# multi-template-matching/MultiTemplateMatching-Python

Measured on AMD Instinct MI355X. Metric: Mpixel-correlations/s, higher is better.
Workload: dtype u8

## Files before the change

include/mtm_hip.h:

```cpp
#ifndef MTM_HIP_H
#define MTM_HIP_H

#include <stddef.h>
#include <stdint.h>

#ifdef __cplusplus
extern "C" {
#endif

#define MTM_ABI_VERSION 9

#define MTM_U8  0
#define MTM_F32 1
#define MTM_U16 2

#define MTM_TM_SQDIFF        0
#define MTM_TM_SQDIFF_NORMED 1
#define MTM_TM_CCORR         2
#define MTM_TM_CCORR_NORMED  3
#define MTM_TM_CCOEFF        4
#define MTM_TM_CCOEFF_NORMED 5

#define MTM_PEAKS_LOCAL  0
#define MTM_PEAKS_GLOBAL 1
// ... 61 lines not shown
    int32_t kernel_used;
    int64_t n_hits;
    int32_t hits_only;
    float   sclk_mhz;
    float   ncc_sum_ms;
    int32_t f32_route;
    int32_t sq_launches;
    float   masked_stat_ms;
    int32_t f32_pieces;
} mtm_timing;

int         mtm_abi_version(void);
int         mtm_device_count(void);
const char* mtm_last_error(void);
int         mtm_ctx_create(mtm_ctx** out, int device_id);
void        mtm_ctx_destroy(mtm_ctx* ctx);
int         mtm_set_option(mtm_ctx* ctx, int option, int64_t value);
int         mtm_get_option(mtm_ctx* ctx, int option, int64_t* value);
#define MTM_POISON_SCRATCH 1
#define MTM_POISON_LDS     2
#define MTM_POISON_ARENAS  4
int         mtm_debug_poison(mtm_ctx* ctx, int pattern_byte, int what);
int         mtm_debug_quotient_check(mtm_ctx* ctx, uint64_t n_cases, uint64_t seed, uint64_t* out4);
void*       mtm_host_alloc(size_t bytes);
void        mtm_host_free(void* p);

int mtm_set_image(mtm_ctx* ctx, const void* px, int rows, int cols, int chans, int dtype,
                  int64_t row_stride_bytes);
int mtm_set_image_downscaled(mtm_ctx* ctx, const void* px, int rows, int cols, int chans, int dtype,
                             int64_t row_stride_bytes, int factor);

int mtm_set_templates(mtm_ctx* ctx, const mtm_templ* templs, int n_templ, int method);

typedef struct mtm_variant {
    int32_t rot90;
    int32_t flip_lr;
    int32_t flip_ud;
    int32_t rows, cols;
    int32_t down;
} mtm_variant;
int mtm_set_templates_augmented(mtm_ctx* ctx, const mtm_templ* bases, int n_bases,
                                const mtm_variant* variants, int n_variants, int method);

int mtm_score_map(mtm_ctx* ctx, int templ_idx, float* out, int64_t out_row_stride_bytes);

int mtm_find_matches(mtm_ctx* ctx, int mode, double score_threshold,
// ... 98 lines not shown
```

multitemplatematching-python_amd/MTM/_lib.py:

```python
import ctypes
import struct
import os
import threading
import weakref

import numpy as np

_HERE = os.path.dirname(os.path.abspath(__file__))
LIB_PATH = os.environ.get("MTM_LIB_PATH") or os.path.join(_HERE, "libmtm_hip.so")

MTM_U8, MTM_F32, MTM_U16 = 0, 1, 2
GROUP_EXCHANGE_HOST, GROUP_EXCHANGE_RCCL = 0, 1
PEAKS_LOCAL, PEAKS_GLOBAL = 0, 1
BORDER_CONSTANT, BORDER_NEAREST = 0, 1
KERNEL_AUTO, KERNEL_NAIVE, KERNEL_DOT4, KERNEL_MFMA = 0, 1, 2, 3
OPT_KERNEL, OPT_PEAK_BORDER, OPT_HIT_CAPACITY, OPT_DOT4_VARIANT, OPT_EXACT_DIV, OPT_HITS_ONLY, OPT_F32_MFMA = 1, 2, 3, 4, 5, 6, 7
OPT_BATCH_MAX_ROWS = 8
OPT_BOXES_MAX_FLOATS = 9
ALL_OPTIONS = (OPT_KERNEL, OPT_PEAK_BORDER, OPT_HIT_CAPACITY, OPT_DOT4_VARIANT, OPT_EXACT_DIV, OPT_HITS_ONLY, OPT_F32_MFMA,
               OPT_BATCH_MAX_ROWS, OPT_BOXES_MAX_FLOATS)
BATCH_MAX_ROWS = 65535
POISON_SCRATCH, POISON_LDS, POISON_ARENAS = 1, 2, 4
E_OVERFLOW = -5
E_HIP = -2
# ... 25 lines not shown

HIT_DTYPE = np.dtype([("templ_idx", "<i4"), ("x", "<i4"), ("y", "<i4"), ("w", "<i4"), ("h", "<i4"),
                      ("score", "<f4")])
BOX_UNIT_DTYPE = np.dtype([("templ_idx", "<i4"), ("y0", "<i4"), ("x0", "<i4"), ("rows", "<i4"), ("cols", "<i4")])
POINT_DTYPE = np.dtype([("templ_idx", "<i4"), ("x", "<i4"), ("y", "<i4")])
assert HIT_DTYPE.itemsize == ctypes.sizeof(MtmHit) == 24
TEMPL_DTYPE = np.dtype([("px", "<u8"), ("mask", "<u8"), ("rows", "<i4"), ("cols", "<i4"), ("chans", "<i4"),
                        ("dtype", "<i4"), ("row_stride", "<i8"), ("mask_row_stride", "<i8")])
assert TEMPL_DTYPE.itemsize == ctypes.sizeof(MtmTempl) == 48
VARIANT_DTYPE = np.dtype([("rot90", "<i4"), ("flip_lr", "<i4"), ("flip_ud", "<i4"), ("rows", "<i4"), ("cols", "<i4"),
                          ("down", "<i4")])

_P = ctypes.POINTER
SYMBOLS = {
    "mtm_abi_version": (ctypes.c_int, []),
    "mtm_device_count": (ctypes.c_int, []),
    "mtm_last_error": (ctypes.c_char_p, []),
    "mtm_ctx_create": (ctypes.c_int, [_P(ctypes.c_void_p), ctypes.c_int]),
    "mtm_ctx_destroy": (None, [ctypes.c_void_p]),
    "mtm_set_option": (ctypes.c_int, [ctypes.c_void_p, ctypes.c_int, ctypes.c_int64]),
    "mtm_get_option": (ctypes.c_int, [ctypes.c_void_p, ctypes.c_int, _P(ctypes.c_int64)]),
    "mtm_debug_poison": (ctypes.c_int, [ctypes.c_void_p, ctypes.c_int, ctypes.c_int]),
    "mtm_debug_quotient_check": (ctypes.c_int, [ctypes.c_void_p, ctypes.c_uint64, ctypes.c_uint64, _P(ctypes.c_uint64)]),
    "mtm_set_image": (ctypes.c_int, [ctypes.c_void_p, ctypes.c_void_p, ctypes.c_int, ctypes.c_int,
                                     ctypes.c_int, ctypes.c_int, ctypes.c_int64]),
    "mtm_set_image_downscaled": (ctypes.c_int, [ctypes.c_void_p, ctypes.c_void_p, ctypes.c_int, ctypes.c_int, ctypes.c_int,
                                                ctypes.c_int, ctypes.c_int64, ctypes.c_int]),
    "mtm_set_templates": (ctypes.c_int, [ctypes.c_void_p, ctypes.c_void_p, ctypes.c_int, ctypes.c_int]),
    "mtm_set_templates_augmented": (ctypes.c_int, [ctypes.c_void_p, ctypes.c_void_p, ctypes.c_int, ctypes.c_void_p, ctypes.c_int,
                                                   ctypes.c_int]),
    "mtm_score_map": (ctypes.c_int, [ctypes.c_void_p, ctypes.c_int, ctypes.c_void_p, ctypes.c_int64]),
    "mtm_find_matches": (ctypes.c_int, [ctypes.c_void_p, ctypes.c_int, ctypes.c_double, ctypes.c_void_p,
                                        ctypes.c_int64, _P(ctypes.c_int64)]),
    "mtm_find_matches_image": (ctypes.c_int, [ctypes.c_void_p, ctypes.c_void_p, ctypes.c_int, ctypes.c_int, ctypes.c_int,
                                              ctypes.c_int, ctypes.c_int64, ctypes.c_int, ctypes.c_double, ctypes.c_void_p,
                                              ctypes.c_int64, _P(ctypes.c_int64)]),
    "mtm_find_matches_image_nms": (ctypes.c_int, [ctypes.c_void_p, ctypes.c_void_p, ctypes.c_int, ctypes.c_int, ctypes.c_int,
                                                  ctypes.c_int, ctypes.c_int64, ctypes.c_double, ctypes.c_double, ctypes.c_int64,
                                                  ctypes.c_void_p, ctypes.c_int64, _P(ctypes.c_int64)]),
    "mtm_find_matches_image_sharded_nms": (ctypes.c_int, [ctypes.c_void_p, ctypes.c_void_p, ctypes.c_int, ctypes.c_int, ctypes.c_int,
                                                          ctypes.c_int, ctypes.c_int64, ctypes.c_double, ctypes.c_double,
                                                          ctypes.c_int64, ctypes.c_int, ctypes.c_void_p, ctypes.c_int,
                                                          ctypes.c_void_p, ctypes.c_int64, _P(ctypes.c_int64)]),
    "mtm_find_matches_batch": (ctypes.c_int, [ctypes.c_void_p, ctypes.c_void_p, ctypes.c_int, ctypes.c_int, ctypes.c_int,
                                              ctypes.c_int, ctypes.c_int, ctypes.c_int64, ctypes.c_int, ctypes.c_double,
                                              ctypes.c_void_p, ctypes.c_int64, ctypes.c_void_p, _P(ctypes.c_int64)]),
# ... 209 lines not shown

class _RecordMemo:
    _rec_key = _rec = _rec_keep = _rec_src = None

    def _records(self, templates):
        if type(templates) is FrozenUnits and templates is self._rec_src and self._rec_key is not None:
            return self._rec
        key = [(id(t), t.shape, id(m)) for t, m in templates]
        if key != self._rec_key:
            self._rec, keep = templ_records(templates)
            self._rec_keep = (keep, [t for t, _ in templates], [m for _, m in templates])
            self._rec_key = key if _zero_copy(templates, keep) else None
        self._rec_src = templates
        return self._rec


_LIVE = weakref.WeakSet()


def live_contexts():
    return [c for c in list(_LIVE) if c._h]


class Context(_RecordMemo):

    def __init__(self, device=None):
        lib = load()
        if device is None:
            device = int(os.environ.get("MTM_DEVICE", os.environ.get("LOCAL_RANK", "0")))
            n = lib.mtm_device_count()
            if n > 0:
                device %= n
        h = ctypes.c_void_p()
        check(lib.mtm_ctx_create(ctypes.byref(h), int(device)), "mtm_ctx_create")
        self._lib = lib
        self._h = h
        self.device = device
        self.lock = threading.RLock()
        self._keep = []
        self._rec_key, self._rec, self._rec_keep = None, None, None
        _LIVE.add(self)
        k = os.environ.get("MTM_KERNEL")
        if k:
            self.set_option(OPT_KERNEL, {"auto": 0, "naive": 1, "dot4": 2, "mfma": 3}[k.lower()])
        b = os.environ.get("MTM_PEAK_BORDER")
        if b:
# ... 383 lines not shown
```

multitemplatematching-python_amd/csrc/mtm_context.hip:

```cpp
#include <cstdio>
#include "mtm_ctx.h"

using namespace mtm;
using namespace mtmi;
#include "mtm_k_image.hip.h"

namespace mtmi {

int prepare_slot(mtm_ctx* c, mtm_ctx::ImageSlot& sl, int src_rows, int src_cols, int chans, int dtype, hipStream_t stream,
                 int factor, SlotGeom* g) {
    (void)c;
    const size_t esz = elem_size(dtype);
    const size_t tight = (size_t)src_cols * chans * esz;
    MTMC(sl.raw.ensure(tight * src_rows));
    const int rows = src_rows / factor, cols = src_cols / factor;
    const int rows_alloc = rows + kPadRows;
    const int pitch = (int)round_up((size_t)cols + kPadCols, 64);
    const size_t f32_bytes = sizeof(float) * pitch * rows_alloc * chans;
    const size_t u8_bytes = (size_t)pitch * rows_alloc * chans;
    const long long geom = (((long long)rows * 65536 + cols) * 8 + chans) * 4 + dtype;
    const size_t caps[3] = {sl.f32.cap, sl.u8.cap, sl.u8b.cap};
    MTMC(sl.f32.ensure(f32_bytes));
    const bool u16_planes = dtype == MTM_U16 && chans == 1;
    const size_t u8b_bytes = u16_planes ? 2 * u8_bytes : u8_bytes;
// ... 257 lines not shown
            if (end == q) break;
            if (x > 0.0 && x <= 1.0 && (f.empty() || x > f.back())) f.push_back(x);
            q = *end == ',' ? end + 1 : end;
        }
        if (!f.empty()) {
            f.back() = 1.0;
            c->upload_bands = f;
        }
    }
    if (const char* v = std::getenv("MTM_CAND_PINNED")) c->cand_pinned = std::atoi(v);
    if (const char* v = std::getenv("MTM_FUSE_LAYOUT")) c->fuse_layout = std::atoi(v);
    if (const char* v = std::getenv("MTM_SEG_SKIP")) c->seg_skip = std::atoi(v);
    if (const char* v = std::getenv("MTM_BAND_MIN_FILL")) c->band_min_fill = std::atof(v);
    if (const char* v = std::getenv("MTM_TEMPL_ON_DEVICE")) c->templ_on_device = std::atoi(v);
    if (const char* v = std::getenv("MTM_ROW_MUX")) c->row_mux = std::atoi(v);
    if (const char* v = std::getenv("MTM_FUSE_STATS")) c->fuse_stats = std::atoi(v);
    if (const char* v = std::getenv("MTM_MFMA_R2")) c->mfma_r2 = std::atoi(v) != 0;
    if (const char* v = std::getenv("MTM_F32_MFMA")) c->f32_mfma = std::atoi(v);
    if (const char* v = std::getenv("MTM_MASKSQ_FUSED")) c->masksq_fused = std::atoi(v);
    if (const char* v = std::getenv("MTM_SPARSE_MAPS")) c->sparse_maps = std::atoi(v);
    if (const char* v = std::getenv("MTM_NMS_DEVICE_MIN")) c->nms_device_min = std::atoll(v) < 0 ? (1ll << 60) : std::max(1, std::atoi(v));
    if (const char* v = std::getenv("MTM_SCREEN_L1")) c->screen_l1 = std::atoi(v);
    if (const char* v = std::getenv("MTM_TAIL_SCREEN")) c->tail_screen = std::atoi(v) != 0;
    if (const char* v = std::getenv("MTM_HOST_TRACE")) c->host_trace = std::atoi(v) != 0;
    if (const char* v = std::getenv("MTM_CLASS_LANES")) c->class_lanes = std::max(1, std::min(8, std::atoi(v)));
    if (const char* v = std::getenv("MTM_COMM_TIMEOUT_S")) c->comm_timeout_s = std::atof(v);
    if (const char* v = std::getenv("MTM_HITS_ONLY")) c->hits_only = std::atoi(v);
    if (const char* v = std::getenv("MTM_EXACT_DIV")) c->exact_div = std::atoi(v);
    {
        hipDeviceProp_t prop;
        if (hipGetDeviceProperties(&prop, c->device) == hipSuccess) c->n_cus = prop.multiProcessorCount;
    }
    if (ensure_copy_stream(c) != MTM_OK) c->copy_stream = nullptr;
    if (c->class_lanes > 1) (void)ensure_lanes(c, 1);
    *out = c;
    return MTM_OK;
}

void mtm_ctx_destroy(mtm_ctx* c) {
    if (!c) return;
    if (c->host_trace) {
        static const char* kPhase[24] = {"entry", "args checked", "templates placed", "call set up", "band 0 copy queued",
                                         "band 0 layout + statistics queued", "band 0 score queued", "last band copy queued",
                                         "last band score queued", "score pass queued", "stream synchronised", "hits verified",
                                         "hits sorted", "(banded: image slot prepared)", "(banded: before the first copy call)", "return",
                                         "(banded: score pass entered)", "(banded: copy stream ready)", "(fm_begin: decisions taken)", "", "", "", "", ""};
// ... 284 lines not shown
```

multitemplatematching-python_amd/csrc/mtm_ctx.h:

```cpp
#pragma once
#include <hip/hip_runtime.h>

#include <algorithm>
#include <chrono>
#include <cmath>
#include <cstdlib>
#include <cstring>
#include <functional>
#include <map>
#include <string>
#include <thread>
#include <tuple>
#include <vector>

#include "mtm_kernels.h"
#include "mtm_mfma_params.h"
#include "mtm_bf16_params.h"
#include "mtm_score_params.h"
#include "mtm_templates_params.h"
#include "mtm_internal.h"

struct ncclComm;

namespace mtmi {
// ... 63 lines not shown
    UnitSrc src{};
    double sum_t = 0.0;
    double mask_ones = 0.0;
    unsigned long long mask_key = 0;
};

struct SizeClass {
    int h = 0, w = 0;
    bool masked = false;
    bool all_u8 = true;
    bool all_u16 = true;
    bool all_f32 = true;
    int kernel = MTM_KERNEL_AUTO;
    int rm_nt = 0, rm_R = 0;
    int kp_nseg = 0;
    struct Slab {
        int r0, r1, c0, c1, ch;
        long long apack_off;
        int tlist_off;
    };
    std::vector<Slab> slabs;
    int slab_nt = 0, slab_R = 0;
    int r2 = 0;
    int tail_split = 0;
    long long mask_rm_off = -1;
    double mask_ones = 0.0;
    int n_pad = 0;
    long long tsum_off = -1;
    std::vector<int> members;
    int tlist_off = 0;
    bool masked_int = false;
    unsigned long long mask_hash = 0;
    long long mask_pack_off = -1;
    bool mask_bf16 = false;
    long long mbf_off_u = -1, mbf_off_v = -1, mbf_group_bytes = 0;
    long long apack_off = 0;
    long long group_bytes = 0;
};

}

namespace mtmi {
struct NmsRequest {
    bool on = false;
    double score_threshold = 0.0, max_overlap = 0.0;
    long long n_object = -1;
// ... 11 lines not shown
    bool sparse = false;
    int flag_tstride = 0, flag_rstride = 0;
    bool seg_skip_used = false;
    bool refine = false;
    bool refine_scan = false;
    bool pp_mode = false;
    bool f32_exact = false;
    bool raw_rig = false;
    float rig_thr = 0.0f;
    float scan_thr = 0.0f;
    float rig_cap = 0.0f;
    int bf16_np = 3;
    bool mbf_thr_on = false;
    bool mbf_global = false;
    float mbf_thr = 0.0f;
    bool mbf_used = false;
    bool cand_pin = false, pin_direct = false, prefetched = false;
    size_t cand_pin_n = 0;
    bool banded_u8 = false;
    bool zero_pending = false;
    bool single_band = false;
    int64_t cand_cap = 0;
    unsigned hash_mask = 0;
    NmsRequest nms;
    long long nms_raw_count = -1;
    long long nms_sure = 0;
};
}

struct mtm_ctx {
    using DevBuf = mtmi::DevBuf;
    using HostTempl = mtmi::HostTempl;
    using SizeClass = mtmi::SizeClass;
    using CallRoute = mtmi::CallRoute;
    using TemplDev = mtm::TemplDev;
    using UnitSrc = mtm::UnitSrc;
    int device = 0;
    hipStream_t stream = nullptr;
    hipEvent_t ev[4] = {nullptr, nullptr, nullptr, nullptr};
    std::vector<std::pair<hipEvent_t, hipEvent_t>> ncc_ev;
    std::vector<std::pair<hipEvent_t, hipEvent_t>> sq_ev;
    int cand_pinned = 1;
    int fuse_layout = 1;
    int lay_r0 = 0, lay_r1 = 0;
    int masksq_fused = 1;

    bool have_image = false;
    int rows = 0, cols = 0, chans = 0, dtype = 0;
    int u8_pitch = 0, f32_pitch = 0, rows_alloc = 0;
    struct ImageSlot {
        DevBuf raw, u8, u8b, f32;
        long long geom = -1;
        bool f32_valid = true;
    } slot[2];
    int cur = 0;
    DevBuf sq_planes;
    bool sq_valid = false;
    hipStream_t copy_stream = nullptr;
    long long nms_device_min = 4096;
    DevBuf nms_buf;
    int sparse_maps = 1;
    DevBuf seg_flags, hits_t;
    hipEvent_t next_ready = nullptr;
    hipStream_t stats_stream = nullptr;
    int screen_l1 = 1;
    int tail_screen = 1;
    int f32_mfma = 1;
    int np1_backoff = 0, np1_backoff_len = 16;
    int seg_skip = 1;
    int templ_on_device = 1;
    int mfma_r2 = 1;
    struct Lane {
        DevBuf stats, stats_rsq, stats_blk, hs1, hs2, raw16, slab_raw, stats_hi, mask_td, sched;
        hipStream_t stream = nullptr;
        hipEvent_t done = nullptr;
        std::vector<hipStream_t> slab_streams;
        std::vector<hipEvent_t> slab_done;
        hipEvent_t slab_fork = nullptr;
    };
    std::vector<Lane> lanes;
    bool slab_fork_early = false;
    hipEvent_t lane_fork = nullptr;
    hipEvent_t f32_built = nullptr;
    int class_lanes = 2;
    std::vector<hipStream_t> slab_streams;
    std::vector<hipEvent_t> slab_done;
    hipEvent_t slab_fork = nullptr;
    std::vector<hipEvent_t> band_ev;
    int banded_cls = -1;
// ... 167 lines not shown
struct BlobTempl {
    int rows, cols, chans, dtype;
    const uint8_t* px;
};
int parse_templ_blob(const std::vector<uint8_t>& b, std::vector<BlobTempl>& out, const char* who, bool u16_ok);
int prepare_window_templates(mtm_ctx* c, const std::vector<BlobTempl>& tl);
int prepare_box_td(mtm_ctx* c, const std::vector<BlobTempl>& tl);
using WindowPeakLaunch = std::function<int(mtm_hit* hits, unsigned long long cap, unsigned long long* counter,
                                           unsigned long long* best, int* nontrivial)>;
int window_peak_pass(mtm_ctx* c, int n, bool global, const WindowPeakLaunch& launch, std::vector<unsigned long long>& best,
                     std::vector<mtm_hit>& recs, const char* who);
int derive_downscaled_u8(mtm_ctx* dst, const mtm_ctx::ImageSlot& src, int src_rows, int src_cols, int chans, int factor,
                         hipStream_t stream);
int check_image_args(const void* px, int rows, int cols, int chans, int dtype, int64_t row_stride_bytes, const char* who);
int ensure_f32_plane(mtm_ctx* c);
int upload_rows_f32c1(mtm_ctx::ImageSlot& sl, const SlotGeom& g, const void* src, int64_t src_stride, int r0, int r1, hipStream_t stream);
int ensure_copy_stream(mtm_ctx* c);
int ensure_lanes(mtm_ctx* c, int n);
int comm_allgather_hits_flagged(mtm_ctx* c, const mtm_hit* local, int64_t n_local, int32_t my_flag, mtm_hit* out,
                                int64_t capacity, int64_t* counts_out, int64_t* n_out, std::vector<int32_t>* flags_out);
int place_templates(mtm_ctx* c);
bool dot_variant_ok(int64_t v);
int launch_stats(mtm_ctx* c, CallRoute& R, const SizeClass& sc, StatPlanes* out, int sb0 = 0, int sb1 = -1);
int launch_ncc(mtm_ctx* c, CallRoute& R, const SizeClass& sc, int list_off, int n_list, const StatPlanes& st, int only_li = -1,
               int yb0 = 0, int yb1 = -1);
int ensure_maps(mtm_ctx* c);
int run_score_all(mtm_ctx* c, CallRoute& R);
bool banded_ok(mtm_ctx* c, const ImageArgs& a, bool* single_band);
int run_score_banded(mtm_ctx* c, CallRoute& R, const ImageArgs& a);
int collect_ncc_time(mtm_ctx* c);

}
```

multitemplatematching-python_amd/csrc/mtm_host.cpp:

```cpp
#include <algorithm>
#include <cmath>
#include <cfloat>
#include <cstring>
#include <numeric>
#include <climits>
#if defined(__SSE2__)
#include <emmintrin.h>
#endif

#include "mtm_internal.h"
#include "mtm_nms_core.h"

namespace mtm {

static thread_local std::string g_last_error;

void set_error(const std::string& msg) { g_last_error = msg; }

void u8_run_sums(const uint8_t* p, size_t n, unsigned long long* sum, unsigned long long* sumsq) {
    unsigned long long s = 0, q = 0;
    size_t i = 0;
#if defined(__SSE2__)
    const __m128i zero = _mm_setzero_si128();
    while (n - i >= 16) {
        const size_t steps = std::min<size_t>((n - i) / 16, 8192);
        __m128i vs = zero, vq = zero;
        for (size_t k = 0; k < steps; ++k, i += 16) {
            const __m128i v = _mm_loadu_si128((const __m128i*)(p + i));
            vs = _mm_add_epi64(vs, _mm_sad_epu8(v, zero));
            const __m128i lo = _mm_unpacklo_epi8(v, zero), hi = _mm_unpackhi_epi8(v, zero);
            vq = _mm_add_epi32(vq, _mm_add_epi32(_mm_madd_epi16(lo, lo), _mm_madd_epi16(hi, hi)));
        }
        alignas(16) unsigned long long ls[2];
        alignas(16) uint32_t lq[4];
        _mm_store_si128((__m128i*)ls, vs);
        _mm_store_si128((__m128i*)lq, vq);
        s += ls[0] + ls[1];
        q += (unsigned long long)lq[0] + lq[1] + lq[2] + lq[3];
    }
#endif
    for (; i < n; ++i) {
        const unsigned v = p[i];
        s += v;
        q += v * v;
    }
    *sum += s;
    *sumsq += q;
}

TemplStats compute_templ_stats(const double* px, const double* mask, int rows, int cols, int chans,
                               int method, bool integer) {
    const size_t plane = (size_t)rows * cols;
    if (mask != nullptr) {
        double s = 0.0;
        for (int c = 0; c < chans; ++c)
            for (size_t i = 0; i < plane; ++i) {
                const double v = px[c * plane + i] * mask[c * plane + i];
                s += v * v;
            }
        return templ_stats_from_sums(nullptr, nullptr, s, true, rows, cols, chans, method);
    }
    double sum[4] = {0, 0, 0, 0}, sumsq[4] = {0, 0, 0, 0};
    for (int c = 0; c < chans && c < 4; ++c) {
        double s = 0.0, sq = 0.0;
        if (integer) {
            long long is = 0, isq = 0;
            for (size_t i = 0; i < plane; ++i) {
                const long long v = (long long)px[c * plane + i];
                is += v;
                isq += v * v;
// ... 358 lines not shown
                    break;
                }
            }
        if (ok) {
            const int32_t slot = (int32_t)kb.size();
            keep.push_back(idx);
            kb.push_back(Kept{b.x, b.y, bx2, by2, barea, -1});
            const size_t cellidx = (size_t)(cy * gw + cx);
            if (tail[cellidx] >= 0) kb[(size_t)tail[cellidx]].next = slot;
            else head[cellidx] = slot;
            tail[cellidx] = slot;
        }
    }
}

}

extern "C" {

const char* mtm_last_error(void) { return mtm::g_last_error.c_str(); }

int mtm_abi_version(void) { return MTM_ABI_VERSION; }

int mtm_nms(const mtm_hit* hits, int64_t n, double score_threshold, int ascending,
            int64_t n_object, double max_overlap, int32_t* keep, int64_t* n_keep) {
    if (n < 0 || (n > 0 && (hits == nullptr || keep == nullptr)) || n_keep == nullptr) {
        mtm::set_error("mtm_nms: bad arguments");
        return MTM_E_INVALID;
    }
    std::vector<float> scores((size_t)n);
    for (int64_t i = 0; i < n; ++i) scores[i] = ascending ? (1.0f - hits[i].score) : hits[i].score;
    const float thr = (float)(ascending ? (1.0 - score_threshold) : score_threshold);
    std::vector<int32_t> kept;
    mtm::nms_boxes(hits, n, scores.data(), thr, (float)max_overlap, kept);
    int64_t m = (int64_t)kept.size();
    if (n_object >= 0 && m > n_object) m = n_object;
    for (int64_t i = 0; i < m; ++i) keep[i] = kept[(size_t)i];
    *n_keep = m;
    return MTM_OK;
}

int mtm_nms_segments(const mtm_hit* hits, const int64_t* seg_counts, int64_t n_seg, double score_threshold, int ascending,
                     double max_overlap, int32_t* keep, int64_t* keep_counts) {
    if (n_seg < 0 || (n_seg > 0 && (seg_counts == nullptr || keep_counts == nullptr))) {
        mtm::set_error("mtm_nms_segments: bad arguments");
        return MTM_E_INVALID;
// ... 37 lines not shown
```

multitemplatematching-python_amd/csrc/mtm_internal.h:

```cpp
#pragma once
#include <cstdint>
#include <string>
#include <vector>

#include "../../include/mtm_hip.h"

namespace mtm {

void set_error(const std::string& msg);

struct TemplStats {
    double mean[4] = {0, 0, 0, 0};
    double templ_norm = 0;
    double templ_sum2 = 0;
    double inv_area = 0;
    int all_ones = 0;
    double templ2_mask2_sum = 0;
    double centred_sum2 = 0;
};

TemplStats compute_templ_stats(const double* px, const double* mask, int rows, int cols, int chans,
                               int method, bool integer);

TemplStats templ_stats_from_sums(const double* sum, const double* sumsq, double templ2_mask2_sum, bool masked, int rows,
                                 int cols, int chans, int method);

void u8_run_sums(const uint8_t* p, size_t n, unsigned long long* sum, unsigned long long* sumsq);

std::vector<int> find_peaks_1d(const float* x, int n, int stride, float height, bool negate);

void line_map_peaks(const float* line, int oh, int ow, float thr, bool mode_min, int templ_idx, int w, int h,
                    std::vector<mtm_hit>& out);

float order_to_float(uint32_t o);

mtm_hit decode_extremum_key(unsigned long long key, bool mode_min, int templ_idx, int ow, int w, int h);
mtm_hit decode_quality_key(unsigned long long key, bool mode_min, int templ_idx, int ow, int w, int h);

int copy_out_hits(const std::vector<mtm_hit>& hits, mtm_hit* out, int64_t capacity, int64_t* n_out, const std::string& msg);
int publish_hits(std::vector<mtm_hit>& hits, std::vector<mtm_hit>& last_hits, mtm_hit* out, int64_t capacity,
                 int64_t* n_out, const std::string& msg);

void nms_boxes(const mtm_hit* hits, int64_t n, const float* scores, float score_threshold,
               float nms_threshold, std::vector<int32_t>& keep);

void nms_select(const mtm_hit* hits, int64_t n, int ascending, float score_threshold, float nms_threshold,
                std::vector<int32_t>& keep, int64_t n_sure = 0);

void sort_hits(std::vector<mtm_hit>& hits, bool mode_min);

// ... 2 lines not shown
```

multitemplatematching-python_amd/csrc/mtm_launch.hip:

```cpp
#include "mtm_ctx.h"

using namespace mtm;
using namespace mtmi;
#include "mtm_k_stats.hip.h"
#include "mtm_k_score.hip.h"
#include "mtm_refine.hip.h"
#include "mtm_maskf32.hip.h"

namespace {

struct DotVariant {
    int px, py, nt;
    bool wide;
    void (*fn)(DotParams, const TemplDev*, const int*, const uint8_t*, StatPlanes, float*);
};
#define DOTV(PX, PY, NT, W) {PX, PY, NT, W, ncc_dot4_kernel<PX, PY, NT, W>}
const DotVariant kDotVariants[] = {
    DOTV(4, 4, 4, false),
    DOTV(4, 4, 2, false),
    DOTV(8, 2, 4, false),
    DOTV(8, 4, 2, false),
    DOTV(4, 2, 4, false),
    DOTV(8, 2, 2, false),
    DOTV(4, 2, 8, false),
// ... 44 lines not shown
    p.only_li = -1;
    return p;
}

int plain_tile_rows(int h) { return std::min(h, kMfChunkH) + kMfRows - 1; }

size_t mfma_lds_layout(MfmaParams& p, int tile_rows, size_t epi_bytes) {
    const size_t lds_main = (std::max<size_t>((size_t)tile_rows * p.lds_pitch, (size_t)kMfRows * epi_bytes) + 15) & ~(size_t)15;
    p.tc_off = (int)lds_main;
    p.st_off = (int)((lds_main + sizeof(MfTemplConst) * 32 + kMfItemBytes + 15) & ~(size_t)15);
    return (size_t)p.st_off;
}

int mfma_row_mux(MfmaParams& p, int R, int nt) {
    p.rm_R = R;
    p.rm_nt = nt;
    while ((1 << p.rm_log2nt) < nt) ++p.rm_log2nt;
    p.rm_steps = p.h + 2 * R - 1;
    p.nyb = (p.oh + 8 * R - 1) / (8 * R);
    p.ntg = 1;
    return rm_tile_rows(p.h, R);
}

int tail_split_for(const mtm_ctx* c, const CallRoute& R, const SizeClass& sc) {
    if (!c->tail_screen || !c->screen_l1 || sc.tail_split <= 0 || sc.r2 != 2 || sc.masked || sc.kernel != MTM_KERNEL_MFMA) return 0;
    if (!R.cand_on || !R.hits_only || R.ext || R.sparse || R.cand_min || c->chans != 1 || c->dtype != MTM_U8) return 0;
    if (c->method != MTM_TM_CCOEFF_NORMED && c->method != MTM_TM_CCORR_NORMED) return 0;
    if (sc.h + 1 > kMfChunkR2 || sc.w > 64) return 0;
    const double thr_lo = (double)R.cand_thr - 1e-6 * std::max(1.0, std::fabs((double)R.cand_thr));
    const double tail = (double)(sc.h - sc.tail_split + 1) / (double)sc.h;
    return thr_lo >= 0.0 && thr_lo - tail >= 0.1 ? sc.tail_split : 0;
}

template <class P>
void wire_candidates(P& p, const mtm_ctx* c, const CallRoute& R, unsigned long long cap) {
    p.cand_on = R.cand_on ? 1 : 0;
    p.hits_only = (p.cand_on && R.hits_only) ? 1 : 0;
    p.cand_min = R.cand_min ? 1 : 0;
    p.cand_thr = R.cand_thr;
    p.cand_cap = cap;
    p.cand_counter = c->cands.as<unsigned long long>();
    p.cand_hits = reinterpret_cast<mtm_hit*>(c->cands.as<uint8_t>() + 16);
}

void wire_mfma_candidates(MfmaParams& p, const mtm_ctx* c, const CallRoute& R, unsigned long long cap) {
    wire_candidates(p, c, R, cap);
    p.cand_thr_lo = (double)R.cand_thr - 1e-6 * std::max(1.0, std::fabs((double)R.cand_thr));
    p.screen_hi = std::min(p.cand_thr_lo, 0.999999) - 1e-6;
    p.sq_floor = 0.99 / std::sqrt((double)p.w * (double)p.h);
    p.screen_l1 = c->screen_l1;
    if (R.cand_pin && p.cand_on && c->pinned) {
        p.cand_pin = reinterpret_cast<mtm_hit*>(static_cast<uint8_t*>(c->pinned) + 16);
        p.cand_pin_n = (unsigned long long)R.cand_pin_n;
    }
// ... 124 lines not shown
    const dim3 g1((ow + 256 * kHsumSeg - 1) / (256 * kHsumSeg), c->rows, c->chans);
    const dim3 g2((ow + 255) / 256, (oh + kVsumBand - 1) / kVsumBand);
    const int want_t = (num_type == 1 || want_t_always) ? 1 : 0;
    const double inv_area = 1.0 / ((double)h * (double)w);
    const bool fused_stats = u8 && c->chans == 1 && w <= 768 && (double)w * h * 65025.0 < 4294967296.0 &&
                             c->fuse_stats;
    if (fused_stats) {
        const int want_sum2 = (!masked_mfma && (num_type == 2 || (normed && num_type != 1) || !want_t_always)) ? 1 : 0;
        const int owg = stats_u8_owg(w);
        const int nsb = (oh + kStatBand4 - 1) / kStatBand4;
        const int b1 = sb1 < 0 ? nsb : std::min(sb1, nsb);
        double* rsq = nullptr;
        if (sc.rm_R > 0 && normed) {
            MTMC(c->stats_rsq.ensure(sizeof(double) * plane));
            rsq = c->stats_rsq.as<double>();
        }
        double* blk = nullptr;
        double* blkq = nullptr;
        int tail_s = 0;
        if (c->chans == 1 && ((sc.r2 > 0 && normed) || (sc.rm_R > 0 && (normed || (masked_mfma && method == MTM_TM_CCORR_NORMED))))) {
            st.blk_pitch = (st.pitch + 15) / 16;
            const size_t nrec = 4 * (size_t)st.blk_pitch * oh;
            tail_s = tail_split_for(c, R, sc);
            MTMC(c->stats_blk.ensure(sizeof(double) * nrec * (tail_s ? 2 : 1)));
            blk = c->stats_blk.as<double>();
            st.blk = blk;
            if (tail_s) {
                blkq = blk + nrec;
                st.blkq = blkq;
            }
        }
        if (b1 > sb0) {
            const dim3 gs((ow + owg - 1) / owg, b1 - sb0);
            StatLayout lay{};
            const uint8_t* src = img.u8;
            int src_pitch = img.u8_pitch;
            if (c->lay_r1 > c->lay_r0) {
                mtm_ctx::ImageSlot& sl = c->slot[c->cur];
                lay.u8 = sl.u8.as<uint8_t>();
                lay.u8b = sl.u8b.as<uint8_t>();
                lay.pitch = img.u8_pitch;
                lay.r0 = c->lay_r0;
                lay.r1 = c->lay_r1;
                src = sl.raw.as<uint8_t>();
                src_pitch = c->cols;
            }
// ... 416 lines not shown
        p.flag_tstride = R.flag_tstride;
        p.flag_rstride = R.flag_rstride;
        const bool normed_m = c->method == MTM_TM_SQDIFF_NORMED || c->method == MTM_TM_CCORR_NORMED || c->method == MTM_TM_CCOEFF_NORMED;
        p.seg_skip = (c->seg_skip && !sc.masked && normed_m) ? 1 : 0;
        R.seg_skip_used = R.seg_skip_used || p.seg_skip != 0;
    }
    int tg0 = 0;
    if (only_li >= 0 && !rm) {
        tg0 = only_li / tgsz;
        p.ntg = 1;
    }
    int tile_rows = r2 ? std::min(h + mb - 1, kMfChunkR2) + (kMfRows - 1) * mb : plain_tile_rows(h);
    if (rm) {
        tile_rows = mfma_row_mux(p, sc.rm_R, sc.rm_nt);
        p.rm_cstride = class_rm_pack_bytes(sc);
        p.rm_rsq = c->stats_rsq.as<double>();
    }
    if (yb1 >= 0) {
        p.yb0 = yb0;
        p.nyb = std::min(yb1, p.nyb) - yb0;
    }
    p.n_work = p.nseg * p.nyb * p.ntg;
    p.tail_split = (r2 && st.blkq != nullptr && only_li < 0 && !p.seg_skip) ? tail_split_for(c, R, sc) : 0;
    const size_t stat_bytes = rm ? 0 : r2 ? (size_t)kMfRows * ((mb + 1) / 2) * 1024 + (p.tail_split ? mf_tail_lds_bytes() : 0)
                                          : (size_t)kMfRows * mf_stat_bytes_per_wave(c->chans == 3 ? 3 : 1);
    const bool ext = R.ext;
    const size_t lds = mfma_ext_or_staging(p, c, ext, mfma_lds_layout(p, tile_rows, kMfEpiBytesPerWave) + stat_bytes);
    p.kp_nseg = sc.kp_nseg;
    p.kp_blocks = sc.kp_nseg ? kp_blocks(h, sc.kp_nseg) : 0;
    const uint8_t* ap = c->apacks.as<uint8_t>() + sc.apack_off +
                        (rm ? (sc.kp_nseg ? 0LL : (long long)sc.rm_R * p.nb * 1024)
                            : (long long)tg0 * (r2 ? 1 : mb) * sc.group_bytes);
    p.n_list = n_all - tg0 * tgsz;
    if (only_li >= 0) p.only_li = only_li - tg0 * tgsz;
    const int* tl_k = c->tlist.as<int>() + sc.tlist_off + tg0 * tgsz;
    MfmaSel sel;
    sel.mb = mb;
    sel.masked = sc.masked;
    sel.rm = rm;
    sel.ch = (c->chans == 3 && !sc.masked) ? 3 : 1;
    sel.method = (c->chans == 1 || sel.ch == 3) ? c->method : -1;
    sel.ext = ext;
    sel.exact_div = c->exact_div != 0 && !(ext && sc.masked);
    sel.r2 = r2;
    sel.kp = sc.kp_nseg > 0;
    const MfmaFn fn = mfma_kernel(sel);
// ... 573 lines not shown
```

multitemplatematching-python_amd/csrc/mtm_mfma.hip.h:

```cpp
#pragma once
#include "mtm_device_util.hip.h"
#include "mtm_mfma_params.h"

namespace mtm {

__device__ __forceinline__ int mf_epi_rot(int j) { return 4 * ((j >> 1) & 3); }
__device__ __forceinline__ int mf_opaque_sgpr(int v) {
    asm volatile("" : "+s"(v));
    return v;
}
template <int METHOD>
__device__ __forceinline__ float finish_vals(int method_rt, double corr, const double (&t)[kMaxChans], double sum2,
                                             double sq, const MfTemplConst& T, int chans) {
    const int method = METHOD >= 0 ? METHOD : method_rt;
    if (T.all_ones) return 1.0f;
    if (method == MTM_TM_CCORR) return (float)corr;
    const int num_type = (method == MTM_TM_CCORR_NORMED) ? 0
                       : (method == MTM_TM_CCOEFF || method == MTM_TM_CCOEFF_NORMED) ? 1 : 2;
    const bool normed = (method == MTM_TM_SQDIFF_NORMED) || (method == MTM_TM_CCORR_NORMED) ||
                        (method == MTM_TM_CCOEFF_NORMED);
    double num = corr;
    if (num_type == 1) {
#pragma unroll
        for (int c = 0; c < kMaxChans; ++c)
// ... 447 lines not shown
#define MTM_R2_STEP_LAST(QA, QB, ACUR, APREV)                               \
                {                                                           \
                    aptr += 1024;                                           \
                    loff += p.lds_pitch;                                    \
                    __builtin_amdgcn_sched_barrier(0);                      \
                    const v4i ar_[2] = {ACUR, APREV};                       \
                    mfma_step2(acc, QA, QB, ar_);                           \
                    __builtin_amdgcn_sched_barrier(0);                      \
                }
#define MTM_R2_FIVE()                                                        \
                MTM_R2_STEP(qx, qy, aA, aC, qx2, qy2, aB)                   \
                MTM_R2_STEP(qx2, qy2, aB, aA, qx, qy, aC)                   \
                MTM_R2_STEP(qx, qy, aC, aB, qx2, qy2, aA)                   \
                MTM_R2_STEP(qx2, qy2, aA, aC, qx, qy, aB)                   \
                MTM_R2_STEP(qx, qy, aB, aA, qx2, qy2, aC)
                MTM_R2_LOAD(qx, qy, aA)
                int ks = 0;
                const int split = (!EXT && kNormed) ? mf_opaque_sgpr(p.tail_split) : 0;
                if (split > 0) {
                    for (; ks + 6 < split; ks += 6) {
                        MTM_R2_FIVE()
                        MTM_R2_STEP(qx2, qy2, aC, aB, qx, qy, aA)
                    }
                    MTM_R2_FIVE()
                    MTM_R2_STEP_LAST(qx2, qy2, aC, aB)
                    ks += 6;
                    asm volatile("s_nop 15\n\ts_nop 15" ::: "memory");
                    bool pass = false;
                    const uint8_t* sbw = smem + p.st_off + wave * 1024 + j * 32;
                    const uint8_t* sbq = sbw + kMfRows * 1024;
                    const MfTailConst* ttl = reinterpret_cast<const MfTailConst*>(smem + p.st_off + 2 * kMfRows * 1024);
#pragma unroll
                    for (int mb = 0; mb < MB; ++mb) {
                        int amax[4] = {INT_MIN, INT_MIN, INT_MIN, INT_MIN};
#pragma unroll
                        for (int c = 0; c < 16; ++c) {
                            const v4i a = acc[mb][c];
                            amax[0] = max(amax[0], a.x);
                            amax[1] = max(amax[1], a.y);
                            amax[2] = max(amax[2], a.z);
                            amax[3] = max(amax[3], a.w);
                        }
                        const double2 s1 = *reinterpret_cast<const double2*>(sbw + mb * 512);
                        const double sq_eff = fmax(*reinterpret_cast<const double*>(sbw + mb * 512 + 16), p.sq_floor);
                        const double2 s1q = *reinterpret_cast<const double2*>(sbq + mb * 512);
                        const double vq = *reinterpret_cast<const double*>(sbq + mb * 512 + 16);
#pragma unroll
                        for (int e = 0; e < 4; ++e) {
                            const MfTemplConst& T = tcl[4 * q + e];
// ... 1109 lines not shown
```

multitemplatematching-python_amd/csrc/mtm_placement.hip:

```cpp
#include <functional>
#include "mtm_ctx.h"

using namespace mtm;
using namespace mtmi;
#include "mtm_templates.hip.h"

namespace {

size_t dot_pack_bytes(int h, int w, int chans) {
    const int w4 = (w + 3) & ~3;
    const int ncy = (h + kDotChunk - 1) / kDotChunk, ncx = (w4 + kDotChunk - 1) / kDotChunk;
    return (size_t)chans * ncy * ncx * kDotChunkBytes;
}

void pack_template_dot4(const HostTempl& t, uint8_t* out) {
    const int h = t.rows, w = t.cols;
    const int w4 = (w + 3) & ~3;
    const int ncy = (h + kDotChunk - 1) / kDotChunk, ncx = (w4 + kDotChunk - 1) / kDotChunk;
    std::memset(out, 0, dot_pack_bytes(h, w, t.chans));
    for (int c = 0; c < t.chans; ++c)
        for (int cy = 0; cy < ncy; ++cy)
            for (int cx = 0; cx < ncx; ++cx) {
                uint8_t* chunk = out + ((size_t)(c * ncy + cy) * ncx + cx) * kDotChunkBytes;
                const int ch = std::min(kDotChunk, h - cy * kDotChunk);
// ... 374 lines not shown
        if (n_cls <= 16) {
            int hs = 0, ws = 0;
            for (const auto& sl : sc.slabs) {
                hs = std::max(hs, sl.r1 - sl.r0);
                ws = std::max(ws, sl.c1 - sl.c0);
            }
            sc.slab_nt = rm_group_templates(n_cls, hs, ws);
            sc.slab_R = 16 / sc.slab_nt;
        }
        return;
    }
    const bool one_pack = c->chans == 1 || (c->chans == 3 && !sc.masked);
    if (c->row_mux && n_cls <= 16 && c->fuse_stats && one_pack && (double)c->chans * sc.w * sc.h * 65025.0 < 4294967296.0) {
        sc.rm_nt = rm_group_templates(n_cls, sc.h, sc.w);
        sc.rm_R = 16 / sc.rm_nt;
    }
    const bool normed = c->method == MTM_TM_SQDIFF_NORMED || c->method == MTM_TM_CCORR_NORMED ||
                        c->method == MTM_TM_CCOEFF_NORMED;
    if (nseg % 4 != 0 && normed && one_pack && (!sc.masked || c->method != MTM_TM_CCOEFF_NORMED))
        sc.kp_nseg = nseg;
    else if (c->mfma_r2 && sc.rm_R == 0 && n_cls > 16 && sc.w <= 64 && c->chans == 1 && !sc.masked &&
             c->method >= MTM_TM_CCORR && c->fuse_stats)
        sc.r2 = 2;
    if (sc.r2 == 2 && sc.h + 1 <= mtm::kMfChunkR2 && sc.h >= 8)
        sc.tail_split = std::max(6, std::min(6 * (int)std::lround(0.65 * sc.h / 6.0), (sc.h - 2) / 6 * 6));
}

size_t place_apacks(const mtm_ctx* c, SizeClass& sc, Bump& a, Bump& ts) {
    const int n_cls = (int)sc.members.size(), groups = mfma_groups_alloc(n_cls);
    size_t bytes = 0;
    switch (sc.kernel) {
        case MTM_KERNEL_MFMA:
            sc.mask_rm_off = -1;
            if (sc.masked && c->row_mux && c->fuse_stats) {
                sc.mask_rm_off = a.take((size_t)rm_pack_bytes(sc.h, sc.w, 16));
                const HostTempl& m0 = c->templs[sc.members[0]];
                sc.mask_ones = m0.on_device ? m0.mask_ones : 0.0;
                if (!m0.on_device)
                    for (double m : m0.mask) sc.mask_ones += m > 0.0 ? 1.0 : 0.0;
            }
            if (!sc.slabs.empty()) {
                sc.apack_off = (long long)a.size;
                for (auto& sl : sc.slabs) {
                    const int hs = sl.r1 - sl.r0, ws = sl.c1 - sl.c0;
                    sl.apack_off = a.take(sc.slab_R > 0 ? (size_t)rm_pack_bytes(hs, ws, sc.slab_R)
                                                        : (size_t)mfma_group_bytes(hs, ws, 1) * groups);
                }
                return 0;
// ... 201 lines not shown
    }
    MTMC(c->td.ensure(sizeof(TemplDev) * n));
    MTMC(c->tlist.ensure(sizeof(int) * std::max<size_t>(1, P.tlist.size())));
    MTMC(c->weights.ensure(sizeof(double) * std::max<size_t>(1, w_off)));
    MTMC(c->packs.ensure(std::max<size_t>(4, p_off)));
    MTMC(c->apacks.ensure(std::max<size_t>(16, a_off) + 16384));
    if (a_off && P.any_host_pack) HIPC(hipMemcpyAsync(c->apacks.p, H.apacks.data(), a_off, hipMemcpyHostToDevice, c->stream));
    HIPC(hipMemcpyAsync(c->td.p, P.td.data(), sizeof(TemplDev) * n, hipMemcpyHostToDevice, c->stream));
    if (!P.tlist.empty())
        HIPC(hipMemcpyAsync(c->tlist.p, P.tlist.data(), sizeof(int) * P.tlist.size(), hipMemcpyHostToDevice, c->stream));
    if (w_off) HIPC(hipMemcpyAsync(c->weights.p, H.wts.data(), sizeof(double) * w_off, hipMemcpyHostToDevice, c->stream));
    if (p_off) HIPC(hipMemcpyAsync(c->packs.p, H.packs.data(), p_off, hipMemcpyHostToDevice, c->stream));
    if (P.any_mbf) {
        MTMC(c->td_u.ensure(sizeof(TemplDev) * n));
        MTMC(c->td_v.ensure(sizeof(TemplDev) * n));
        HIPC(hipMemcpyAsync(c->td_u.p, P.td_u.data(), sizeof(TemplDev) * n, hipMemcpyHostToDevice, c->stream));
        HIPC(hipMemcpyAsync(c->td_v.p, P.td_v.data(), sizeof(TemplDev) * n, hipMemcpyHostToDevice, c->stream));
    }
    MTMC(c->tsum.ensure(sizeof(double) * std::max<size_t>(2, ts_off)));
    if (ts_off) HIPC(hipMemcpyAsync(c->tsum.p, H.tsums.data(), sizeof(double) * ts_off, hipMemcpyHostToDevice, c->stream));
    for (size_t k = 0; k < P.classes.size(); ++k)
        if (P.dev_pack[k]) MTMC(pack_class_on_device(c, P.classes[k]));
    for (const SizeClass& sc : P.classes)
        if (sc.tail_split > 0 && sc.kernel == MTM_KERNEL_MFMA && !sc.members.empty()) {
            hipLaunchKernelGGL(tail_consts_kernel, dim3((unsigned)sc.members.size()), dim3(64), 0, c->stream,
                               c->apacks.as<uint8_t>() + sc.apack_off, sc.group_bytes, sc.h, sc.w, sc.tail_split,
                               c->tlist.as<int>() + sc.tlist_off, c->td.as<TemplDev>());
            HIPC(hipGetLastError());
        }
    const bool local_sources = P.any_host_pack || P.any_mbf || w_off || p_off || ts_off || new_units;
    if (local_sources) HIPC(hipStreamSynchronize(c->stream));
    c->place_pending = !local_sources;
    drain.armed = false;
    if (new_units) c->usrc_host.swap(P.units);
    c->classes.swap(P.classes);
    c->td_host.swap(P.td);
    c->tlist_host.swap(P.tlist);
    c->list2d.swap(P.list2d);
    c->list2d_off = P.list2d_off;
    c->maps_floats = P.maps.size;
    c->placed = true;
    return MTM_OK;
}

}

namespace mtmi {

int place_templates(mtm_ctx* c) {
    if (!c->have_image || !c->have_templ) {
        set_error("set the image and the templates first");
        return MTM_E_STATE;
    }
    if (c->placed) return MTM_OK;
    if (c->place_pending) {
        HIPC(hipStreamSynchronize(c->stream));
        c->place_pending = false;
    }
    Placement P;
    MTMC(plan_placement(c, P));
    for (int i : P.host_px) MTMC(ensure_host_pixels(c, i));
    HostArenas H;
    pack_on_host(c, P, H);
    return upload_placement(c, P, H);
}

int parse_templ_blob(const std::vector<uint8_t>& b, std::vector<BlobTempl>& out, const char* who, bool u16_ok) {
    size_t off = 0;
    auto rd = [&](void* dst, size_t n) {
        if (off + n > b.size()) return false;
// ... 500 lines not shown
```

Before: 381,900.

## Choose tail-split depth per call from a statistical bound on threshold and size

Replaces the fixed 65%-of-height tail split with a rule that picks the earliest split row where the remaining tail cannot reach the candidate threshold within a z-scaled sigma bound. The split is cached per route and per threshold. Tail constants are relaunched lazily when the chosen split differs from the one placed. The MFMA r2 loop now steps one row at a time up to the split instead of in fixed 6-row groups, so the split can stop earlier. The aim is to screen candidates sooner and skip full correlation work, at the risk of a looser loop, extra constant-kernel launches, and reliance on the statistical bound being safe.

```diff
diff --git a/include/mtm_hip.h b/include/mtm_hip.h
--- a/include/mtm_hip.h
+++ b/include/mtm_hip.h
@@ -107,6 +107,7 @@
 #define MTM_POISON_ARENAS  4
 int         mtm_debug_poison(mtm_ctx* ctx, int pattern_byte, int what);
 int         mtm_debug_quotient_check(mtm_ctx* ctx, uint64_t n_cases, uint64_t seed, uint64_t* out4);
+int         mtm_debug_tail_split(int h, int w, double thr);
 void*       mtm_host_alloc(size_t bytes);
 void        mtm_host_free(void* p);
 
diff --git a/multitemplatematching-python_amd/MTM/_lib.py b/multitemplatematching-python_amd/MTM/_lib.py
--- a/multitemplatematching-python_amd/MTM/_lib.py
+++ b/multitemplatematching-python_amd/MTM/_lib.py
@@ -71,6 +71,7 @@
     "mtm_get_option": (ctypes.c_int, [ctypes.c_void_p, ctypes.c_int, _P(ctypes.c_int64)]),
     "mtm_debug_poison": (ctypes.c_int, [ctypes.c_void_p, ctypes.c_int, ctypes.c_int]),
     "mtm_debug_quotient_check": (ctypes.c_int, [ctypes.c_void_p, ctypes.c_uint64, ctypes.c_uint64, _P(ctypes.c_uint64)]),
+    "mtm_debug_tail_split": (ctypes.c_int, [ctypes.c_int, ctypes.c_int, ctypes.c_double]),
     "mtm_set_image": (ctypes.c_int, [ctypes.c_void_p, ctypes.c_void_p, ctypes.c_int, ctypes.c_int,
                                      ctypes.c_int, ctypes.c_int, ctypes.c_int64]),
     "mtm_set_image_downscaled": (ctypes.c_int, [ctypes.c_void_p, ctypes.c_void_p, ctypes.c_int, ctypes.c_int, ctypes.c_int,
@@ -326,6 +327,10 @@
     return [c for c in list(_LIVE) if c._h]
 
 
+def debug_tail_split(h, w, thr):
+    return int(load().mtm_debug_tail_split(int(h), int(w), float(thr)))
+
+
 class Context(_RecordMemo):
 
     def __init__(self, device=None):
diff --git a/multitemplatematching-python_amd/csrc/mtm_context.hip b/multitemplatematching-python_amd/csrc/mtm_context.hip
--- a/multitemplatematching-python_amd/csrc/mtm_context.hip
+++ b/multitemplatematching-python_amd/csrc/mtm_context.hip
@@ -303,6 +303,7 @@
     if (const char* v = std::getenv("MTM_NMS_DEVICE_MIN")) c->nms_device_min = std::atoll(v) < 0 ? (1ll << 60) : std::max(1, std::atoi(v));
     if (const char* v = std::getenv("MTM_SCREEN_L1")) c->screen_l1 = std::atoi(v);
     if (const char* v = std::getenv("MTM_TAIL_SCREEN")) c->tail_screen = std::atoi(v) != 0;
+    if (const char* v = std::getenv("MTM_TAIL_SPLIT")) c->tail_split_force = std::max(0, std::atoi(v));
     if (const char* v = std::getenv("MTM_HOST_TRACE")) c->host_trace = std::atoi(v) != 0;
     if (const char* v = std::getenv("MTM_CLASS_LANES")) c->class_lanes = std::max(1, std::min(8, std::atoi(v)));
     if (const char* v = std::getenv("MTM_COMM_TIMEOUT_S")) c->comm_timeout_s = std::atof(v);
diff --git a/multitemplatematching-python_amd/csrc/mtm_ctx.h b/multitemplatematching-python_amd/csrc/mtm_ctx.h
--- a/multitemplatematching-python_amd/csrc/mtm_ctx.h
+++ b/multitemplatematching-python_amd/csrc/mtm_ctx.h
@@ -109,6 +109,7 @@
     std::vector<Slab> slabs;
     int slab_nt = 0, slab_R = 0;
     int r2 = 0;
+    bool tail_ok = false;
     int tail_split = 0;
     long long mask_rm_off = -1;
     double mask_ones = 0.0;
@@ -166,6 +167,8 @@
     bool single_band = false;
     int64_t cand_cap = 0;
     unsigned hash_mask = 0;
+    int tail_h = 0, tail_w = 0, tail_s = 0;
+    float tail_thr = 0.0f;
     NmsRequest nms;
     long long nms_raw_count = -1;
     long long nms_sure = 0;
@@ -209,6 +212,8 @@
     hipStream_t stats_stream = nullptr;
     int screen_l1 = 1;
     int tail_screen = 1;
+    int tail_split_force = 0;
+    std::vector<int> tail_valid;
     int f32_mfma = 1;
     int np1_backoff = 0, np1_backoff_len = 16;
     int seg_skip = 1;
@@ -422,6 +427,7 @@
 int place_templates(mtm_ctx* c);
 bool dot_variant_ok(int64_t v);
 int launch_stats(mtm_ctx* c, CallRoute& R, const SizeClass& sc, StatPlanes* out, int sb0 = 0, int sb1 = -1);
+int launch_tail_consts(mtm_ctx* c, const SizeClass& sc, int split, hipStream_t stream);
 int launch_ncc(mtm_ctx* c, CallRoute& R, const SizeClass& sc, int list_off, int n_list, const StatPlanes& st, int only_li = -1,
                int yb0 = 0, int yb1 = -1);
 int ensure_maps(mtm_ctx* c);
diff --git a/multitemplatematching-python_amd/csrc/mtm_host.cpp b/multitemplatematching-python_amd/csrc/mtm_host.cpp
--- a/multitemplatematching-python_amd/csrc/mtm_host.cpp
+++ b/multitemplatematching-python_amd/csrc/mtm_host.cpp
@@ -46,6 +46,16 @@
     }
     *sum += s;
     *sumsq += q;
+}
+
+int tail_split_rule(int h, int w, double thr_lo) {
+    if (!(thr_lo >= 0.0) || h < 8 || w < 1) return 0;
+    for (int s = 6; s <= h - 2; ++s) {
+        const double tail = (double)(h - s + 1) / (double)h;
+        const double sigma = std::sqrt((double)s / (double)h) / std::sqrt((double)w * (double)h);
+        if (thr_lo - tail >= kTailSplitZ * sigma) return (double)s / (double)h <= kTailSplitMaxFrac ? s : 0;
+    }
+    return 0;
 }
 
 TemplStats compute_templ_stats(const double* px, const double* mask, int rows, int cols, int chans,
@@ -450,6 +460,8 @@
 
 int mtm_abi_version(void) { return MTM_ABI_VERSION; }
 
+int mtm_debug_tail_split(int h, int w, double thr) { return mtm::tail_split_rule(h, w, thr); }
+
 int mtm_nms(const mtm_hit* hits, int64_t n, double score_threshold, int ascending,
             int64_t n_object, double max_overlap, int32_t* keep, int64_t* n_keep) {
     if (n < 0 || (n > 0 && (hits == nullptr || keep == nullptr)) || n_keep == nullptr) {
diff --git a/multitemplatematching-python_amd/csrc/mtm_internal.h b/multitemplatematching-python_amd/csrc/mtm_internal.h
--- a/multitemplatematching-python_amd/csrc/mtm_internal.h
+++ b/multitemplatematching-python_amd/csrc/mtm_internal.h
@@ -26,6 +26,10 @@
                                  int cols, int chans, int method);
 
 void u8_run_sums(const uint8_t* p, size_t n, unsigned long long* sum, unsigned long long* sumsq);
+int tail_split_rule(int h, int w, double thr_lo);
+constexpr double kTailSplitZ = 6.5;
+constexpr double kTailSplitMaxFrac = 0.94;
+constexpr double kTailDefaultThr = 0.5;
 
 std::vector<int> find_peaks_1d(const float* x, int n, int stride, float height, bool negate);
 
diff --git a/multitemplatematching-python_amd/csrc/mtm_launch.hip b/multitemplatematching-python_amd/csrc/mtm_launch.hip
--- a/multitemplatematching-python_amd/csrc/mtm_launch.hip
+++ b/multitemplatematching-python_amd/csrc/mtm_launch.hip
@@ -90,14 +90,31 @@
     return rm_tile_rows(p.h, R);
 }
 
-int tail_split_for(const mtm_ctx* c, const CallRoute& R, const SizeClass& sc) {
-    if (!c->tail_screen || !c->screen_l1 || sc.tail_split <= 0 || sc.r2 != 2 || sc.masked || sc.kernel != MTM_KERNEL_MFMA) return 0;
+int tail_split_for(const mtm_ctx* c, CallRoute& R, const SizeClass& sc) {
+    if (!c->tail_screen || !c->screen_l1 || !sc.tail_ok || sc.r2 != 2 || sc.masked || sc.kernel != MTM_KERNEL_MFMA) return 0;
     if (!R.cand_on || !R.hits_only || R.ext || R.sparse || R.cand_min || c->chans != 1 || c->dtype != MTM_U8) return 0;
     if (c->method != MTM_TM_CCOEFF_NORMED && c->method != MTM_TM_CCORR_NORMED) return 0;
     if (sc.h + 1 > kMfChunkR2 || sc.w > 64) return 0;
     const double thr_lo = (double)R.cand_thr - 1e-6 * std::max(1.0, std::fabs((double)R.cand_thr));
-    const double tail = (double)(sc.h - sc.tail_split + 1) / (double)sc.h;
-    return thr_lo >= 0.0 && thr_lo - tail >= 0.1 ? sc.tail_split : 0;
+    if (!(thr_lo >= 0.0)) return 0;
+    if (c->tail_split_force > 0) return std::max(6, std::min(c->tail_split_force, sc.h - 2));
+    if (R.tail_h != sc.h || R.tail_w != sc.w || R.tail_thr != R.cand_thr) {
+        R.tail_s = tail_split_rule(sc.h, sc.w, thr_lo);
+        R.tail_h = sc.h;
+        R.tail_w = sc.w;
+        R.tail_thr = R.cand_thr;
+    }
+    return R.tail_s;
+}
+
+static int ensure_tail_consts(mtm_ctx* c, const SizeClass& sc, int split) {
+    if (split <= 0 || sc.members.empty()) return MTM_OK;
+    const bool mine = !c->classes.empty() && &sc >= c->classes.data() && &sc < c->classes.data() + c->classes.size();
+    const size_t k = mine ? (size_t)(&sc - c->classes.data()) : 0;
+    if (mine && k < c->tail_valid.size() && c->tail_valid[k] == split) return MTM_OK;
+    MTMC(launch_tail_consts(c, sc, split, c->stream));
+    if (mine && k < c->tail_valid.size()) c->tail_valid[k] = split;
+    return MTM_OK;
 }
 
 template <class P>
@@ -268,6 +285,7 @@
             st.blk_pitch = (st.pitch + 15) / 16;
             const size_t nrec = 4 * (size_t)st.blk_pitch * oh;
             tail_s = tail_split_for(c, R, sc);
+            MTMC(ensure_tail_consts(c, sc, tail_s));
             MTMC(c->stats_blk.ensure(sizeof(double) * nrec * (tail_s ? 2 : 1)));
             blk = c->stats_blk.as<double>();
             st.blk = blk;
@@ -730,6 +748,7 @@
     }
     p.n_work = p.nseg * p.nyb * p.ntg;
     p.tail_split = (r2 && st.blkq != nullptr && only_li < 0 && !p.seg_skip) ? tail_split_for(c, R, sc) : 0;
+    MTMC(ensure_tail_consts(c, sc, p.tail_split));
     const size_t stat_bytes = rm ? 0 : r2 ? (size_t)kMfRows * ((mb + 1) / 2) * 1024 + (p.tail_split ? mf_tail_lds_bytes() : 0)
                                           : (size_t)kMfRows * mf_stat_bytes_per_wave(c->chans == 3 ? 3 : 1);
     const bool ext = R.ext;
diff --git a/multitemplatematching-python_amd/csrc/mtm_mfma.hip.h b/multitemplatematching-python_amd/csrc/mtm_mfma.hip.h
--- a/multitemplatematching-python_amd/csrc/mtm_mfma.hip.h
+++ b/multitemplatematching-python_amd/csrc/mtm_mfma.hip.h
@@ -493,9 +493,17 @@
                         MTM_R2_FIVE()
                         MTM_R2_STEP(qx2, qy2, aC, aB, qx, qy, aA)
                     }
-                    MTM_R2_FIVE()
-                    MTM_R2_STEP_LAST(qx2, qy2, aC, aB)
-                    ks += 6;
+#pragma nounroll
+                    for (; ks + 1 < split; ++ks) {
+                        MTM_R2_STEP(qx, qy, aA, aC, qx2, qy2, aB)
+                        aC = aA;
+                        aA = aB;
+                        qx = qx2;
+                        qy = qy2;
+                    }
+                    MTM_R2_STEP_LAST(qx, qy, aA, aC)
+                    aC = aA;
+                    ks = split;
                     asm volatile("s_nop 15\n\ts_nop 15" ::: "memory");
                     bool pass = false;
                     const uint8_t* sbw = smem + p.st_off + wave * 1024 + j * 32;
diff --git a/multitemplatematching-python_amd/csrc/mtm_placement.hip b/multitemplatematching-python_amd/csrc/mtm_placement.hip
--- a/multitemplatematching-python_amd/csrc/mtm_placement.hip
+++ b/multitemplatematching-python_amd/csrc/mtm_placement.hip
@@ -420,8 +420,19 @@
     else if (c->mfma_r2 && sc.rm_R == 0 && n_cls > 16 && sc.w <= 64 && c->chans == 1 && !sc.masked &&
              c->method >= MTM_TM_CCORR && c->fuse_stats)
         sc.r2 = 2;
-    if (sc.r2 == 2 && sc.h + 1 <= mtm::kMfChunkR2 && sc.h >= 8)
-        sc.tail_split = std::max(6, std::min(6 * (int)std::lround(0.65 * sc.h / 6.0), (sc.h - 2) / 6 * 6));
+    if (sc.r2 == 2 && sc.h + 1 <= mtm::kMfChunkR2 && sc.h >= 8) {
+        sc.tail_ok = true;
+        sc.tail_split = c->tail_split_force > 0 ? std::max(6, std::min(c->tail_split_force, sc.h - 2))
+                                                : tail_split_rule(sc.h, sc.w, kTailDefaultThr - 1e-6);
+    }
+}
+
+int queue_tail_consts(mtm_ctx* c, const SizeClass& sc, int split, hipStream_t stream) {
+    hipLaunchKernelGGL(tail_consts_kernel, dim3((unsigned)sc.members.size()), dim3(64), 0, stream,
+                       c->apacks.as<uint8_t>() + sc.apack_off, sc.group_bytes, sc.h, sc.w, split,
+                       c->tlist.as<int>() + sc.tlist_off, c->td.as<TemplDev>());
+    HIPC(hipGetLastError());
+    return MTM_OK;
 }
 
 size_t place_apacks(const mtm_ctx* c, SizeClass& sc, Bump& a, Bump& ts) {
@@ -669,18 +680,19 @@
     for (size_t k = 0; k < P.classes.size(); ++k)
         if (P.dev_pack[k]) MTMC(pack_class_on_device(c, P.classes[k]));
     for (const SizeClass& sc : P.classes)
-        if (sc.tail_split > 0 && sc.kernel == MTM_KERNEL_MFMA && !sc.members.empty()) {
-            hipLaunchKernelGGL(tail_consts_kernel, dim3((unsigned)sc.members.size()), dim3(64), 0, c->stream,
-                               c->apacks.as<uint8_t>() + sc.apack_off, sc.group_bytes, sc.h, sc.w, sc.tail_split,
-                               c->tlist.as<int>() + sc.tlist_off, c->td.as<TemplDev>());
-            HIPC(hipGetLastError());
-        }
+        if (sc.tail_split > 0 && sc.kernel == MTM_KERNEL_MFMA && !sc.members.empty())
+            MTMC(queue_tail_consts(c, sc, sc.tail_split, c->stream));
     const bool local_sources = P.any_host_pack || P.any_mbf || w_off || p_off || ts_off || new_units;
     if (local_sources) HIPC(hipStreamSynchronize(c->stream));
     c->place_pending = !local_sources;
     drain.armed = false;
     if (new_units) c->usrc_host.swap(P.units);
     c->classes.swap(P.classes);
+    c->tail_valid.assign(c->classes.size(), 0);
+    for (size_t k = 0; k < c->classes.size(); ++k) {
+        const SizeClass& sc = c->classes[k];
+        if (sc.tail_split > 0 && sc.kernel == MTM_KERNEL_MFMA && !sc.members.empty()) c->tail_valid[k] = sc.tail_split;
+    }
     c->td_host.swap(P.td);
     c->tlist_host.swap(P.tlist);
     c->list2d.swap(P.list2d);
@@ -693,6 +705,8 @@
 }
 
 namespace mtmi {
+
+int launch_tail_consts(mtm_ctx* c, const SizeClass& sc, int split, hipStream_t stream) { return queue_tail_consts(c, sc, split, stream); }
 
 int place_templates(mtm_ctx* c) {
     if (!c->have_image || !c->have_templ) {
```

Result: faster. 405,200, median of 6 (+6.1%).
